# Ighina/MultimodalTopicSegmentation

Hardware: AMD Instinct MI355X
Metric: sentences/sec (fwd+bwd) (higher is better)
Workload: dtype bf16; 1 GPU; BASELINE configs[1]: restricted-window transformer tagger d=1792 heads=8 ff=256 radius=15 layers=1 focal loss, 64 docs x 256 sentences per GPU, fwd+bwd+Adam(eps 1e-7), inputs resident in HBM; global_batch_docs=64, sentences_per_doc=256, parallelism=dp1 (document-sharded, RCCL all-reduce)

## Files before the change

multimodaltopicsegmentation_amd/csrc/gemm.hip:

```cpp
#include <algorithm>
#include <math.h>
#include <stdlib.h>
#include "common.h"

#include "gemm_common.h"


template <int LAYOUT, typename TC, bool GLDS>
__global__ __launch_bounds__(256, 2) void gemm_bf16_kernel(const GemmArgs a) {
  constexpr bool A_KMAJOR = (LAYOUT == MTS_NT || LAYOUT == MTS_NN);
  constexpr bool B_KMAJOR = (LAYOUT == MTS_NT || LAYOUT == MTS_TT);
  extern __shared__ __attribute__((aligned(16))) char smem[];

  const int tid = threadIdx.x;
  const int lane = tid & 63;
  const int wave = tid >> 6;
  const int wm = wave >> 1, wn = wave & 1;
  const int r16 = lane & 15, g = lane >> 4;

  const int ntn = (a.N + BN - 1) / BN;
  const int ntm = (a.M + BM - 1) / BM;
  const int nt = ntn * ntm;
  int bid = xcd_remap(blockIdx.x, nt);
  const int bm0 = (ntm < ntn ? bid % ntm : bid / ntn) * BM;
// ... 485 lines not shown
  if (accumulate) load4<float>(C + (size_t)m * ldc + n, s);
  const size_t plane = (size_t)M * N;
  for (int z = 0; z < splits; ++z) {
    float v[4];
    load4<float>(slab + z * plane + (size_t)m * N + n, v);
#pragma unroll
    for (int i = 0; i < 4; ++i) s[i] += v[i];
  }
  store4<float>(C + (size_t)m * ldc + n, s);
}

__global__ __launch_bounds__(256) void splitk_reduce_t_kernel(const float* __restrict__ slab, int splits, int M, int N, float* __restrict__ Ct,
                                                              int ldc, int accumulate) {
  __shared__ float tile[32][33];
  const int n0 = blockIdx.x * 32, m0 = blockIdx.y * 32;
  const int tx = threadIdx.x & 31, ty = threadIdx.x >> 5;
  const size_t plane = (size_t)M * N;
#pragma unroll
  for (int r = ty; r < 32; r += 8) {
    const int m = m0 + r, n = n0 + tx;
    float s = 0.f;
    if (m < M && n < N) {
      const float* p = slab + (size_t)m * N + n;
      int z = 0;
      for (; z + 7 < splits; z += 8) {
        float v[8];
#pragma unroll
        for (int u = 0; u < 8; ++u) v[u] = p[(size_t)(z + u) * plane];
#pragma unroll
        for (int u = 0; u < 8; ++u) s += v[u];
      }
      for (; z < splits; ++z) s += p[(size_t)z * plane];
    }
    tile[r][tx] = s;
  }
  __syncthreads();
#pragma unroll
  for (int r = ty; r < 32; r += 8) {
    const int n = n0 + r, m = m0 + tx;
    if (n < N && m < M) {
      float* o = Ct + (size_t)n * ldc + m;
      *o = accumulate ? *o + tile[tx][r] : tile[tx][r];
    }
  }
}

template <typename T> __global__ void cast_kernel(const float* __restrict__ src, T* __restrict__ dst, size_t n) {
  size_t i = ((size_t)blockIdx.x * blockDim.x + threadIdx.x) * 4;
  const size_t stride = (size_t)gridDim.x * blockDim.x * 4;
  for (; i + 3 < n; i += stride) {
    float v[4];
    load4<float>(src + i, v);
    store4<T>(dst + i, v);
  }
  if (i < n && i + 3 >= n)
    for (size_t j = i; j < n; ++j) dst[j] = from_f32<T>(src[j]);
}

template <typename T> __global__ void cast_concat_kernel(const float* __restrict__ s1, const float* __restrict__ s2, T* __restrict__ dst,
                                                          size_t rows, int D1, int D2) {
  const int D = D1 + D2, q = D / 4;
  const size_t total = rows * q;
  for (size_t i = (size_t)blockIdx.x * blockDim.x + threadIdx.x; i < total; i += (size_t)gridDim.x * blockDim.x) {
    const size_t r = i / q;
    const int e = (int)(i - r * q) * 4;
    float v[4];
    load4<float>(e < D1 ? s1 + r * D1 + e : s2 + r * D2 + (e - D1), v);
    store4<T>(dst + r * D + e, v);
  }
}

extern "C" int mts_cast_concat(void* stream, int dst_dtype, size_t rows, int D1, int D2, const float* src1, const float* src2, void* dst) {
  MTS_CHECK_ARG(src1 && src2 && dst && D1 > 0 && D2 > 0 && D1 % 4 == 0 && D2 % 4 == 0, "mts_cast_concat: bad arguments (widths must be multiples of 4)");
  if (rows == 0) return MTS_OK;
  const int blocks = (int)std::min<size_t>(4096, (rows * ((D1 + D2) / 4) + 255) / 256);
  if (dst_dtype == MTS_BF16) hipLaunchKernelGGL(cast_concat_kernel<bf16_t>, dim3(blocks), dim3(256), 0, (hipStream_t)stream, src1, src2, (bf16_t*)dst, rows, D1, D2);
  else if (dst_dtype == MTS_F32) hipLaunchKernelGGL(cast_concat_kernel<float>, dim3(blocks), dim3(256), 0, (hipStream_t)stream, src1, src2, (float*)dst, rows, D1, D2);
  else { mts_set_error("mts_cast_concat: bad dtype %d", dst_dtype); return MTS_ERR_INVALID; }
  MTS_LAUNCH_CHECK("mts_cast_concat");
  return MTS_OK;
}

extern "C" size_t mts_colsum_workspace(int N) { return (size_t)COLSUM_RS * (size_t)N * sizeof(float); }

extern "C" int mts_colsum(void* stream, int dtype, int M, int N, const void* X, int ldx, float* out, int accumulate,
                          void* partial) {
  MTS_CHECK_ARG(M > 0 && N > 0 && X && out && partial, "mts_colsum: bad arguments");
  MTS_CHECK_ARG(dtype == MTS_F32 || dtype == MTS_BF16, "mts_colsum: bad dtype %d", dtype);
  MTS_CHECK_ARG(ldx % 4 == 0, "mts_colsum: ldx must be a multiple of 4");
  hipStream_t st = (hipStream_t)stream;
  const int nparts = min(COLSUM_RS, M);
  dim3 grid(ceil_div(N, 64), COLSUM_RS);
  (void)nparts;
  if (dtype == MTS_F32)
    hipLaunchKernelGGL(colsum_partial_kernel<float>, grid, dim3(256), 0, st, (const float*)X, M, N, ldx, (float*)partial);
  else
    hipLaunchKernelGGL(colsum_partial_kernel<bf16_t>, grid, dim3(256), 0, st, (const bf16_t*)X, M, N, ldx, (float*)partial);
  hipLaunchKernelGGL(colsum_final_kernel, dim3(ceil_div(N, 64)), dim3(256), 0, st, (const float*)partial, N, COLSUM_RS, out,
                     accumulate);
  MTS_LAUNCH_CHECK("mts_colsum");
  return MTS_OK;
}

extern "C" int mts_cast(void* stream, int dst_dtype, const float* src, void* dst, size_t n) {
  MTS_CHECK_ARG(src && dst, "mts_cast: null pointer");
  if (n == 0) return MTS_OK;
  hipStream_t st = (hipStream_t)stream;
  const int blocks = (int)std::min<size_t>(2048, (n / 4 + 255) / 256 + 1);
  if (dst_dtype == MTS_BF16)
    hipLaunchKernelGGL(cast_kernel<bf16_t>, dim3(blocks), dim3(256), 0, st, src, (bf16_t*)dst, n);
  else if (dst_dtype == MTS_F32)
    hipLaunchKernelGGL(cast_kernel<float>, dim3(blocks), dim3(256), 0, st, src, (float*)dst, n);
  else {
    mts_set_error("mts_cast: bad dtype %d", dst_dtype);
    return MTS_ERR_INVALID;
  }
  MTS_LAUNCH_CHECK("mts_cast");
  return MTS_OK;
}

int mts_launch_gemm256(const GemmArgs& a, int layout, bool c_is_f32, int splits, hipStream_t st);
int mts_launch_gemm224(const GemmArgs& a, int layout, bool c_is_f32, int splits, hipStream_t st);
bool mts_gemm224t_applies(const GemmArgs& a, int layout, bool c_is_f32, int splits);

static thread_local int g_gemm_glds = -1;
static thread_local int g_tile_mode = -1;
static thread_local int g_force_splits = 0;
static thread_local int g_tile_order = 1;
static thread_local int g_gemm_deep = 1;
static thread_local int g_chain = 0;
static thread_local int g_combine = 0;
#define MTS_GEMM_WS_HEAD 8192
static thread_local int g_last_tile = 0, g_last_splits = 0;

static thread_local void (*g_mid_hook)(void) = nullptr;
extern "C" int mts_gemm_set_mid_hook(void (*fn)(void)) { g_mid_hook = fn; return MTS_OK; }

extern "C" int mts_gemm_last_plan(int* tile, int* splits) {
  if (tile) *tile = g_last_tile;
  if (splits) *splits = g_last_splits;
  return MTS_OK;
}

void mts_band_set_mfma(int on);
void mts_band_set_fused(int on);
void mts_full_set_mfma(int on);
void mts_t5_set_mfma(int on);
static thread_local int g_f32_mfma = 1;
static thread_local int g_big_min_k = 256;
static thread_local int g_gemm_variant = 0;
void mts_lstm_pair_set_spin_limit(int n);
void mts_lstm_pair_set_max_pairs(int n);
void mts_lstm_pair_set_parts(int n);
extern "C" int mts_set_option(const char* key, int value) {
  if (!key) return MTS_ERR_INVALID;
  if (!strcmp(key, "gemm_tile")) { g_tile_mode = value; return MTS_OK; }
  if (!strcmp(key, "gemm_glds")) { g_gemm_glds = value; return MTS_OK; }
  if (!strcmp(key, "gemm_splits")) { g_force_splits = value; return MTS_OK; }
  if (!strcmp(key, "gemm_order")) { g_tile_order = value; return MTS_OK; }
  if (!strcmp(key, "gemm_chain")) { g_chain = value; return MTS_OK; }
  if (!strcmp(key, "gemm_combine")) { g_combine = value; return MTS_OK; }
  if (!strcmp(key, "gemm_deep")) { g_gemm_deep = value; return MTS_OK; }
  if (!strcmp(key, "gemm_variant")) { g_gemm_variant = value; return MTS_OK; }
  if (!strcmp(key, "gemm_big_min_k")) { g_big_min_k = value; return MTS_OK; }
  if (!strcmp(key, "gemm_f32_mfma")) { g_f32_mfma = value; return MTS_OK; }
  if (!strcmp(key, "band_mfma")) { mts_band_set_mfma(value); return MTS_OK; }
  if (!strcmp(key, "band_fused_bwd")) { mts_band_set_fused(value); return MTS_OK; }
  if (!strcmp(key, "full_mfma")) { mts_full_set_mfma(value); return MTS_OK; }
  if (!strcmp(key, "t5_mfma")) { mts_t5_set_mfma(value); return MTS_OK; }
  if (!strcmp(key, "lstm_pair_spin_limit")) { mts_lstm_pair_set_spin_limit(value); return MTS_OK; }
  if (!strcmp(key, "lstm_pair_max_pairs")) { mts_lstm_pair_set_max_pairs(value); return MTS_OK; }
  if (!strcmp(key, "lstm_parts")) { mts_lstm_pair_set_parts(value); return MTS_OK; }
  mts_set_error("mts_set_option: unknown key %s", key);
  return MTS_ERR_INVALID;
}

template <int LAYOUT, typename TC>
static void launch_bf16(const GemmArgs& a, int splits, hipStream_t st) {
  const int nt = ceil_div(a.M, BM) * ceil_div(a.N, BN);
  if (g_gemm_glds < 0) {
    const char* e = getenv("MTS_GEMM_GLDS");
    g_gemm_glds = (e && e[0] == '0') ? 0 : 1;
  }
  const bool glds = g_gemm_glds && (a.K % BK == 0) && (a.ksplit % BK == 0) && a.M >= 8 && a.N >= 8;
  if (glds) {
    GemmArgs b = a;
    const bool deep = g_gemm_deep && (size_t)nt * splits <= 256 && a.ksplit >= 4 * BK;
    b.nbuf = deep ? 4 : 2;
    auto k = gemm_bf16_kernel<LAYOUT, TC, true>;
    if (deep && mts_dyn_lds(k, 8 * TILE_BYTES, "gemm") != MTS_OK) b.nbuf = 2;
    hipLaunchKernelGGL(k, dim3(nt, 1, splits), dim3(256), (b.nbuf == 4 ? 8 : 4) * TILE_BYTES, st, b);
  } else {
    hipLaunchKernelGGL((gemm_bf16_kernel<LAYOUT, TC, false>), dim3(nt, 1, splits), dim3(256), 4 * TILE_BYTES, st, a);
  }
}

static void plan_bf16(int c_dtype, int layout, int M, int N, int K, unsigned epilogue, bool has_workspace, size_t workspace_bytes,
                      int* use256_out, int* splits_out) {
  if (g_tile_mode < 0) {
    const char* e = getenv("MTS_GEMM_TILE");
    g_tile_mode = e ? atoi(e) : 0;
  }
  const int tile_mode = g_tile_mode;
  const unsigned plain = epilogue & ~MTS_EPI_ACCUM;
  const bool can_split = (c_dtype == MTS_F32 && plain == 0 && has_workspace && N % 4 == 0 && K >= 2048);
  const bool can256 = (K % BK == 0) && K >= g_big_min_k && M >= 8 && N >= 8 && tile_mode != 128;
  const double bw = 3500.0;
  double best = 1e30;
  int splits = 1;
  int use256 = 0;
  const bool can224 = can256 && (N % 224 == 0) && tile_mode != 256;
  for (int big = 0; big <= (can256 ? 2 : 0); ++big) {
    if (big == 2 && !can224) continue;
    if (tile_mode == 256 && can256 && big != 1) continue;
    if (tile_mode == 224 && can224 && big != 2) continue;
    const int tile = big ? 256 : 128;
    const double slots = big ? 256.0 : 512.0;
    const double t_k = layout == MTS_TN ? (big == 2 ? (M % 256 == 0 ? 0.0160 : 0.0200) : big == 1 ? 0.0218 : 0.0145)
                                        : (big ? 0.0232 * (big == 2 ? 0.875 : 1.0) : 0.0180);
    const double t_0 = big ? 7.7 : 6.5;
    const int nt = ceil_div(M, tile) * (big == 2 ? N / 224 : ceil_div(N, tile));
    for (int sp = 1; sp <= (can_split ? 32 : 1); ++sp) {
      const int ks = ceil_div(ceil_div(K, sp), BK) * BK;
      if (ceil_div(K, ks) != sp) continue;
      if (sp > 1 && (size_t)sp * M * N * sizeof(float) > workspace_bytes) break;
      if (g_force_splits > 0 && can_split && sp != g_force_splits) continue;
      const double rounds = ceil((double)nt * sp / slots);
      const double cost = rounds * (ks * t_k + t_0) + (sp > 1 ? (2.0 * sp + 1.0) * M * N * 4.0 / 1e6 / bw : 0.0);
      if (cost < best) { best = cost; splits = sp; use256 = big; }
    }
  }
  *use256_out = use256;
  *splits_out = splits;
}

int mts_gemm224_last_kernel();
int mts_launch_gemm224t_pair(const GemmArgs& a, int splits, const void* A2, const void* B2, float* slab2, hipStream_t st);
bool mts_gemm224t_applies(const GemmArgs& a, int layout, bool c_is_f32, int splits);

static int wgrad_pair_splits(int M, int N, int K, size_t workspace_bytes) {
  if (M % 256 || N % 224 || K % 64 || K < 256) return -1;
  static int cus = 0;
  if (!cus) { int dev = 0; hipDeviceProp_t pr; cus = (hipGetDevice(&dev) == hipSuccess && hipGetDeviceProperties(&pr, dev) == hipSuccess) ? pr.multiProcessorCount : 256; }
  const int nt = (M / 256) * (N / 224);
  int sp = std::max(1, std::min(32, cus / (2 * nt)));
  for (; sp >= 1; --sp) {
    const int ks = ceil_div(ceil_div(K, sp), BK) * BK;
    if (ceil_div(K, ks) != sp) continue;
    if (ks >= 128 && K - (sp - 1) * ks >= 128 && (size_t)2 * sp * M * N * sizeof(float) <= workspace_bytes) return sp;
  }
  return -1;
}
extern "C" size_t mts_wgrad_pair_workspace(int M, int N, int K) {
  const int sp = wgrad_pair_splits(M, N, K, (size_t)-1);
  return sp < 1 ? 0 : (size_t)2 * sp * M * N * sizeof(float);
}
extern "C" int mts_wgrad_pair(void* stream, int M, int N, int K, const void* A1, const void* B1, float* C1, int ldc1, const void* A2, const void* B2,
                              float* C2t, int ldc2t, int lda, int ldb, int accumulate, void* workspace, size_t workspace_bytes) {
  MTS_CHECK_ARG(M > 0 && N > 0 && K > 0 && A1 && B1 && C1 && A2 && B2 && C2t && workspace, "mts_wgrad_pair: bad arguments");
  MTS_CHECK_ARG(ldc1 >= N && ldc2t >= M && ldc1 % 4 == 0, "mts_wgrad_pair: bad output strides");
  const int sp = wgrad_pair_splits(M, N, K, workspace_bytes);
  MTS_UNSUPPORTED(sp >= 1, "mts_wgrad_pair: M=%d N=%d K=%d not covered (M %% 256, N %% 224, K %% 64) or workspace too small", M, N, K);
  hipStream_t st = (hipStream_t)stream;
  GemmArgs a;
  memset(&a, 0, sizeof(a));
  a.A = A1; a.B = B1; a.C = C1;
  a.M = M; a.N = N; a.K = K; a.lda = lda; a.ldb = ldb; a.ldc = ldc1;
  a.epi = 0; a.colscale = 1.0f;
  a.ksplit = ceil_div(ceil_div(K, sp), BK) * BK;
  a.order = 1; a.nbuf = 2; a.variant = 0;
  float* const planes = (float*)workspace;
  a.slab = planes;
  float* const planes2 = planes + (size_t)sp * M * N;
  MTS_UNSUPPORTED(mts_gemm224t_applies(a, MTS_TN, true, sp), "mts_wgrad_pair: operands not covered by the four-wave weight-gradient kernel (alignment / strides)");
  const int rc = mts_launch_gemm224t_pair(a, sp, A2, B2, planes2, st);
  MTS_UNSUPPORTED(rc == MTS_OK, "mts_wgrad_pair: launch refused");
  hipLaunchKernelGGL(splitk_reduce_kernel, dim3((unsigned)(((size_t)M * (N / 4) + 255) / 256)), dim3(256), 0, st, (const float*)planes, sp, M, N, C1, ldc1,
                     accumulate ? 1 : 0);
  hipLaunchKernelGGL(splitk_reduce_t_kernel, dim3(ceil_div(N, 32), ceil_div(M, 32)), dim3(256), 0, st, (const float*)planes2, sp, M, N, C2t, ldc2t,
                     accumulate ? 1 : 0);
  MTS_LAUNCH_CHECK("mts_wgrad_pair");
  return MTS_OK;
}

extern "C" int mts_gemm_plan(int a_dtype, int c_dtype, int layout, int M, int N, int K, unsigned epilogue, size_t workspace_bytes,
                             int* tile, int* splits) {
  MTS_CHECK_ARG(M > 0 && N > 0 && K > 0, "mts_gemm_plan: bad shape M=%d N=%d K=%d", M, N, K);
  MTS_CHECK_ARG(layout == MTS_NT || layout == MTS_NN || layout == MTS_TN || layout == MTS_TT, "mts_gemm_plan: bad layout %d", layout);
  MTS_CHECK_ARG(a_dtype == MTS_F32 || a_dtype == MTS_BF16, "mts_gemm_plan: bad a_dtype %d", a_dtype);
  int use256 = 0, sp = 1;
  const size_t ws_planes = workspace_bytes > MTS_GEMM_WS_HEAD ? workspace_bytes - MTS_GEMM_WS_HEAD : 0;
  if (a_dtype == MTS_BF16) plan_bf16(c_dtype, layout, M, N, K, epilogue, ws_planes > 0, ws_planes, &use256, &sp);
  if (tile) *tile = a_dtype == MTS_F32 ? (g_f32_mfma ? 128 : 64) : use256 == 2 ? 224 : use256 == 1 ? 256 : 128;
  if (splits) *splits = sp;
  return MTS_OK;
}

extern "C" int mts_gemm(void* stream, int a_dtype, int c_dtype, int layout, int M, int N, int K, const void* A, int lda,
                        const void* B, int ldb, void* C, int ldc, const float* bias, const void* residual, int ldr,
                        void* aux, int ldaux, unsigned epilogue, float colscale, int ncols_scaled, void* workspace, size_t workspace_bytes) {
  MTS_CHECK_ARG(M > 0 && N > 0 && K > 0, "mts_gemm: bad shape M=%d N=%d K=%d", M, N, K);
  MTS_CHECK_ARG(A && B && C, "mts_gemm: null operand");
  MTS_CHECK_ARG(layout == MTS_NT || layout == MTS_NN || layout == MTS_TN || layout == MTS_TT, "mts_gemm: bad layout %d", layout);
  MTS_CHECK_ARG(a_dtype == MTS_F32 || a_dtype == MTS_BF16, "mts_gemm: bad a_dtype %d", a_dtype);
  MTS_CHECK_ARG(c_dtype == MTS_F32 || c_dtype == a_dtype, "mts_gemm: c_dtype must be f32 or a_dtype");
  MTS_CHECK_ARG(!(epilogue & MTS_EPI_BIAS) || bias, "mts_gemm: MTS_EPI_BIAS without bias");
  MTS_CHECK_ARG(!(epilogue & MTS_EPI_RESIDUAL) || residual, "mts_gemm: MTS_EPI_RESIDUAL without residual");
  MTS_CHECK_ARG(!(epilogue & MTS_EPI_ACCUM) || c_dtype == MTS_F32, "mts_gemm: MTS_EPI_ACCUM needs fp32 C");
// ... 102 lines not shown
```

multimodaltopicsegmentation_amd/csrc/norm.hip:

```cpp
#include <algorithm>
#include <type_traits>
#include "common.h"
#include "loss_elems.h"

#define ROW_WAVES 4
#define BWD_MAX_BLOCKS 512

template <typename T, int NV> struct RowRegs {
  float v[NV][4];
  __device__ __forceinline__ void load(const T* row, int D, int lane) {
#pragma unroll
    for (int i = 0; i < NV; ++i) {
      const int e = 4 * (lane + 64 * i);
      if (e < D) load4<T>(row + e, v[i]);
      else { v[i][0] = v[i][1] = v[i][2] = v[i][3] = 0.f; }
    }
  }
  __device__ __forceinline__ void store(T* row, int D, int lane) const {
#pragma unroll
    for (int i = 0; i < NV; ++i) {
      const int e = 4 * (lane + 64 * i);
      if (e < D) store4<T>(row + e, v[i]);
    }
  }
  __device__ __forceinline__ void zero() {
#pragma unroll
    for (int i = 0; i < NV; ++i) v[i][0] = v[i][1] = v[i][2] = v[i][3] = 0.f;
  }
};

template <int NV> __device__ __forceinline__ void row_stats(const float (&x)[NV][4], int D, int lane, float& mean, float& rstd, float eps) {
  float s = 0.f;
#pragma unroll
  for (int i = 0; i < NV; ++i) s += (x[i][0] + x[i][1]) + (x[i][2] + x[i][3]);
  mean = wave_sum(s) / (float)D;
  float q = 0.f;
#pragma unroll
  for (int i = 0; i < NV; ++i) {
    if (4 * (lane + 64 * i) < D) {
#pragma unroll
      for (int j = 0; j < 4; ++j) { const float d = x[i][j] - mean; q += d * d; }
    }
  }
  rstd = 1.0f / sqrtf(wave_sum(q) / (float)D + eps);
}

template <typename T, int NV, int EMBED, bool FULL = false>
__global__ __launch_bounds__(64 * ROW_WAVES) void ln_fwd_kernel(
    const void* __restrict__ xin, const float* __restrict__ pos, int pos_offset, int L, const float* __restrict__ type0,
    const float* __restrict__ gamma, const float* __restrict__ beta, float eps, int rows, int D,
    T* __restrict__ y, T* __restrict__ pre, float* __restrict__ mean_out, float* __restrict__ rstd_out,
    const float* __restrict__ head_w, const float* __restrict__ head_b, int n_out, float* __restrict__ scores,
    const int32_t* __restrict__ row_src, const float* __restrict__ xin2 = nullptr, int D1 = 0) {
  const int lane = threadIdx.x & 63;
  const int row = blockIdx.x * ROW_WAVES + (threadIdx.x >> 6);
  if (row >= rows) return;
  float gv[NV][4], bv[NV][4];
#pragma unroll
  for (int i = 0; i < NV; ++i) {
    const int e = 4 * (lane + 64 * i);
    if (FULL || e < D) { load4<float>(gamma + e, gv[i]); load4<float>(beta + e, bv[i]); }
  }
  float x[NV][4];
  if constexpr (EMBED) {
    const int src = row_src ? row_src[row] : row;
    const int Dx = xin2 ? D1 : D;
    const float* xr = reinterpret_cast<const float*>(xin) + (size_t)src * Dx;
    const float* xr2 = xin2 ? xin2 + (size_t)src * (D - D1) - D1 : xr;
    const float* pr = pos + (size_t)(pos_offset + src % L) * D;
#pragma unroll
    for (int i = 0; i < NV; ++i) {
      const int e = 4 * (lane + 64 * i);
      if (FULL || e < D) {
        float a[4], b[4], c[4];
        if constexpr (EMBED == 2) load4<bf16_t>(reinterpret_cast<const bf16_t*>(xin) + (size_t)src * D + e, a);
        else load4<float>((e < Dx ? xr : xr2) + e, a);
        load4<float>(pr + e, b); load4<float>(type0 + e, c);
#pragma unroll
        for (int j = 0; j < 4; ++j) x[i][j] = (a[j] + b[j]) + c[j];
        if constexpr (sizeof(T) == 2) {
#pragma unroll
          for (int j = 0; j < 4; ++j) x[i][j] = to_f32(from_f32<T>(x[i][j]));
        }
      } else { x[i][0] = x[i][1] = x[i][2] = x[i][3] = 0.f; }
    }
    if (pre) {
#pragma unroll
      for (int i = 0; i < NV; ++i) { const int e = 4 * (lane + 64 * i); if (FULL || e < D) store4<T>(pre + (size_t)row * D + e, x[i]); }
    }
  } else {
    const T* xr = reinterpret_cast<const T*>(xin) + (size_t)row * D;
#pragma unroll
    for (int i = 0; i < NV; ++i) {
      const int e = 4 * (lane + 64 * i);
      if (FULL || e < D) load4<T>(xr + e, x[i]);
      else { x[i][0] = x[i][1] = x[i][2] = x[i][3] = 0.f; }
    }
  }
  float mean, rstd;
  row_stats<NV>(x, D, lane, mean, rstd, eps);
  float hs[4] = {0.f, 0.f, 0.f, 0.f};
  const float* hwp = head_w ? head_w : gamma;
  const int hw_max = head_w ? n_out - 1 : 0;
#pragma unroll
  for (int i = 0; i < NV; ++i) {
    const int e = 4 * (lane + 64 * i);
    if (FULL || e < D) {
#pragma unroll
      for (int j = 0; j < 4; ++j) x[i][j] = (x[i][j] - mean) * rstd * gv[i][j] + bv[i][j];
      if (head_w) {
#pragma unroll
        for (int c = 0; c < 4; ++c) {
          float w[4];
          load4<float>(hwp + (size_t)min(c, hw_max) * D + e, w);
#pragma unroll
          for (int j = 0; j < 4; ++j) hs[c] += to_f32(from_f32<T>(x[i][j])) * w[j];
        }
      }
    }
  }
  if (y) {
#pragma unroll
    for (int i = 0; i < NV; ++i) {
      const int e = 4 * (lane + 64 * i);
      if (FULL || e < D) store4<T>(y + (size_t)row * D + e, x[i]);
    }
  }
  if (lane == 0 && mean_out) { mean_out[row] = mean; rstd_out[row] = rstd; }
  if (head_w) {
    for (int c = 0; c < n_out; ++c) {
      const float s = wave_sum(hs[c]);
      if (lane == 0) scores[(size_t)row * n_out + c] = s + head_b[c];
    }
  }
}

template <typename T>
__global__ __launch_bounds__(64 * ROW_WAVES) void head_fwd_kernel(const T* __restrict__ x, int ldx, int rows, int D, int n_out,
                                                                const float* __restrict__ w, const float* __restrict__ b,
                                                                float* __restrict__ scores) {
  const int lane = threadIdx.x & 63;
  const int row = blockIdx.x * ROW_WAVES + (threadIdx.x >> 6);
  if (row >= rows) return;
  float hs[4] = {0.f, 0.f, 0.f, 0.f};
  for (int e = 4 * lane; e < D; e += 256) {
    float xv[4];
    load4<T>(x + (size_t)row * ldx + e, xv);
    for (int c = 0; c < n_out; ++c) {
      float wv[4];
      load4<float>(w + (size_t)c * D + e, wv);
#pragma unroll
      for (int j = 0; j < 4; ++j) hs[c] += xv[j] * wv[j];
    }
  }
  for (int c = 0; c < n_out; ++c) {
    const float s = wave_sum(hs[c]);
    if (lane == 0) scores[(size_t)row * n_out + c] = s + b[c];
  }
}

template <typename T>
__global__ __launch_bounds__(256) void head_bwd_data_kernel(const float* __restrict__ ds, const float* __restrict__ w, int rows, int D,
                                                            int n_out, T* __restrict__ dx, int lddx, int accumulate) {
  const size_t idx = (size_t)blockIdx.x * 256 + threadIdx.x;
  const int per_row = D / 4;
  const size_t total = (size_t)rows * per_row;
  if (idx >= total) return;
  const int row = (int)(idx / per_row);
  const int e = 4 * (int)(idx % per_row);
  float o[4] = {0.f, 0.f, 0.f, 0.f};
  if (accumulate) load4<T>(dx + (size_t)row * lddx + e, o);
  for (int c = 0; c < n_out; ++c) {
    const float s = ds[(size_t)row * n_out + c];
    float wv[4];
    load4<float>(w + (size_t)c * D + e, wv);
#pragma unroll
    for (int j = 0; j < 4; ++j) o[j] += s * wv[j];
  }
  store4<T>(dx + (size_t)row * lddx + e, o);
}

struct EmbArgs { int B, L, Bc, nchunks; const int32_t* row0; const int32_t* lengths; float* dpos_part; };

template <typename T, int NV, bool WIDE, bool FULL = false, int NHG = 0, bool EMB = false>
__global__ __launch_bounds__(64 * ROW_WAVES, 2) void ln_bwd_kernel(
    const T* __restrict__ x, const T* __restrict__ dy_, const float* __restrict__ dlogit, const float* __restrict__ head_w, int n_out,
    const float* __restrict__ gamma, const float* __restrict__ mean, const float* __restrict__ rstd, int rows, int D,
    T* __restrict__ dx, float* __restrict__ partial, const EmbArgs ea) {
  static_assert(!(EMB && (WIDE || NHG > 0)), "the embedding form has no head and D <= 2048");
  constexpr bool HG = NHG > 0;
  constexpr int NR = HG ? NHG + 1 : EMB ? 2 : 3;
  constexpr int NS = HG ? NHG + 2 : NR;
  constexpr int NA = HG ? NHG : 2;
  const T* __restrict__ dy = HG ? nullptr : dy_;
  __shared__ float red[ROW_WAVES][NR][64 * 4];
  __shared__ __attribute__((aligned(16))) float gam_s[NV * 256];
  __shared__ __attribute__((aligned(16))) float hw_s[EMB ? 1 : 4][EMB ? 4 : NV * 256];
  __shared__ __attribute__((aligned(16))) float task_s[EMB ? ROW_WAVES : 1][EMB ? NV * 256 : 4];
  const int lane = threadIdx.x & 63;
  const int wave = __builtin_amdgcn_readfirstlane(threadIdx.x >> 6);
  const int col0 = WIDE ? (int)blockIdx.y * (NV * 256) : 0;
  for (int idx = threadIdx.x; idx < NV * 256; idx += 64 * ROW_WAVES) {
    const int e = col0 + idx;
    gam_s[idx] = (e < D) ? gamma[e] : 0.f;
    if constexpr (!EMB) {
      if (head_w)
        for (int c = 0; c < n_out; ++c) hw_s[c][idx] = (e < D) ? head_w[(size_t)c * D + e] : 0.f;
    }
  }
  __syncthreads();
  float acc[NA][NV][4];
  float dxs[NV][4];
  float tsum[HG ? NHG : 1];
#pragma unroll
  for (int i = 0; i < NV; ++i)
#pragma unroll
    for (int j = 0; j < 4; ++j) {
      dxs[i][j] = 0.f;
#pragma unroll
      for (int c = 0; c < NA; ++c) acc[c][i][j] = 0.f;
    }
#pragma unroll
  for (int c = 0; c < (HG ? NHG : 1); ++c) tsum[c] = 0.f;
  if constexpr (EMB) {
#pragma unroll
    for (int i = 0; i < NV; ++i) *reinterpret_cast<float4*>(&task_s[wave][4 * (lane + 64 * i)]) = make_float4(0.f, 0.f, 0.f, 0.f);
  }

  const float invD = 1.0f / (float)D;
  const int stride = gridDim.x * ROW_WAVES;
  Pack<T, 4> px[NV], pd[HG ? 1 : NV];
  float mu_n = 0.f, rs_n = 0.f, dl_n[4] = {0.f, 0.f, 0.f, 0.f};
  const float* dlp = head_w ? dlogit : mean;
  const int dl_mul = head_w ? n_out : 1, dl_max = head_w ? n_out - 1 : 0;
  auto fetch = [&](int r) {
    mu_n = mean[r];
    rs_n = rstd[r];
    if constexpr (!EMB) {
#pragma unroll
      for (int c = 0; c < 4; ++c) dl_n[c] = dlp[(size_t)r * dl_mul + min(c, dl_max)];
    }
#pragma unroll
    for (int i = 0; i < NV; ++i) {
      const int e = col0 + 4 * (lane + 64 * i);
      if (FULL || e < D) {
        px[i].load(x + (size_t)r * D + e);
        if constexpr (!HG) { if (dy) pd[i].load(dy + (size_t)r * D + e); }
      }
    }
  };
  int task = blockIdx.x * ROW_WAVES + wave;
  int ti = 0, tb = 0, tbend = 0;
  const int ntasks = EMB ? ea.L * ea.nchunks : 0;
  auto row_at = [&](int b, int i) { return ea.row0 ? ea.row0[b] + i : b * ea.L + i; };
  auto valid = [&](int b, int i) { return !ea.row0 || i < ea.lengths[b]; };
  auto open_task = [&](int t) {
    ti = t % ea.L;
    tb = (t / ea.L) * ea.Bc;
    tbend = min(ea.B, tb + ea.Bc);
    while (tb < tbend && !valid(tb, ti)) ++tb;
    return tb < tbend;
  };
  auto write_task = [&](int t) {
    float* o = ea.dpos_part + (size_t)t * D;
#pragma unroll
    for (int i = 0; i < NV; ++i) {
      const int e = 4 * (lane + 64 * i);
      float4* slot = reinterpret_cast<float4*>(&task_s[EMB ? wave : 0][EMB ? e : 0]);
      const float4 v = *slot;
      if (FULL || e < D) *reinterpret_cast<float4*>(o + e) = v;
      *slot = make_float4(0.f, 0.f, 0.f, 0.f);
    }
  };
  auto skip_empty_tasks = [&]() {
    if constexpr (EMB) {
      while (task < ntasks && !open_task(task)) task += stride;
    }
  };
  int row;
  if constexpr (EMB) { skip_empty_tasks(); row = task < ntasks ? row_at(tb, ti) : -1; }
  else row = task < rows ? task : -1;
  if (row >= 0) fetch(row);
  while (row >= 0) {
    const float mu = mu_n, rs = rs_n;
    float xh[NV][4], gy[NV][4];
// ... 516 lines not shown
  float dbs[4] = {0.f, 0.f, 0.f, 0.f};
  Pack<T, 4> px[NV];
  float dl_n[4] = {0.f, 0.f, 0.f, 0.f};
  auto fetch = [&](int r) {
#pragma unroll
    for (int c = 0; c < 4; ++c) dl_n[c] = ds[(size_t)r * n_out + min(c, n_out - 1)];
#pragma unroll
    for (int i = 0; i < NV; ++i) {
      const int e = col0 + 4 * (lane + 64 * i);
      if (FULL || e < D) px[i].load(x + (size_t)r * ldx + e);
    }
  };
  const int stride = gridDim.x * ROW_WAVES;
  int row = blockIdx.x * ROW_WAVES + wave;
  if (row < rows) fetch(row);
  for (; row < rows; row += stride) {
    float dl[4], xv[NV][4];
#pragma unroll
    for (int c = 0; c < 4; ++c) dl[c] = (c < n_out) ? dl_n[c] : 0.f;
#pragma unroll
    for (int i = 0; i < NV; ++i) {
      const int e = col0 + 4 * (lane + 64 * i);
#pragma unroll
      for (int j = 0; j < 4; ++j) xv[i][j] = (FULL || e < D) ? px[i].get(j) : 0.f;
    }
    if (row + stride < rows) fetch(row + stride);
#pragma unroll
    for (int c = 0; c < 4; ++c) dbs[c] += dl[c];
#pragma unroll
    for (int i = 0; i < NV; ++i)
#pragma unroll
      for (int c = 0; c < 4; ++c)
#pragma unroll
        for (int j = 0; j < 4; ++j) dw[c][i][j] += dl[c] * xv[i][j];
  }
  float* slab = partial + (size_t)blockIdx.x * 5 * D;
#pragma unroll
  for (int i = 0; i < NV; ++i) {
    __syncthreads();
#pragma unroll
    for (int c = 0; c < 4; ++c)
#pragma unroll
      for (int j = 0; j < 4; ++j) red[wave][c][lane * 4 + j] = dw[c][i][j];
    __syncthreads();
    for (int t = threadIdx.x; t < 4 * 256; t += 64 * ROW_WAVES) {
      const int slot = t / 256, col = t % 256;
      const int e = col0 + 256 * i + col;
      if (e < D) {
        float s = 0.f;
#pragma unroll
        for (int w = 0; w < ROW_WAVES; ++w) s += red[w][slot][col];
        slab[(size_t)slot * D + e] = s;
      }
    }
  }
  __syncthreads();
  if (lane == 0)
    for (int c = 0; c < 4; ++c) red[wave][c][0] = dbs[c];
  __syncthreads();
  if (threadIdx.x < 4) {
    float s = 0.f;
    for (int w = 0; w < ROW_WAVES; ++w) s += red[w][threadIdx.x][0];
    slab[(size_t)4 * D + threadIdx.x] = s;
  }
}

#define SR_COLS 32
struct SlabOuts { float* o[6]; int short_slot, short_len; const float* alt; int alt_slot, alt_nb; };
__global__ __launch_bounds__(256) void slab_reduce_kernel(const float* __restrict__ partial, int nblocks, int nslots, int D, const SlabOuts so) {
  __shared__ float4 red[32][8];
  const int c4 = threadIdx.x & 7, grp = threadIdx.x >> 3;
  const int e = blockIdx.x * SR_COLS + 4 * c4;
  const int slot = blockIdx.y;
  float* o = so.o[slot];
  if (!o) return;
  if (slot == so.alt_slot) { partial = so.alt - (size_t)slot * D; nblocks = so.alt_nb; nslots = 1; }
  const int len = (slot == so.short_slot) ? so.short_len : D;
  float4 s = make_float4(0.f, 0.f, 0.f, 0.f);
  if (e < len) {
    const float* p = partial + (size_t)slot * D + e;
    const size_t bs = (size_t)nslots * D;
    int b = grp;
    for (; b + 32 * 7 < nblocks; b += 32 * 8) {
      float4 v[8];
#pragma unroll
      for (int u = 0; u < 8; ++u) v[u] = *reinterpret_cast<const float4*>(p + (size_t)(b + 32 * u) * bs);
#pragma unroll
      for (int u = 0; u < 8; ++u) { s.x += v[u].x; s.y += v[u].y; s.z += v[u].z; s.w += v[u].w; }
    }
    for (; b < nblocks; b += 32) {
      const float4 v = *reinterpret_cast<const float4*>(p + (size_t)b * bs);
      s.x += v.x; s.y += v.y; s.z += v.z; s.w += v.w;
    }
  }
  red[grp][c4] = s;
  __syncthreads();
  if (grp == 0 && e < len) {
    float4 t = red[0][c4];
#pragma unroll
    for (int gidx = 1; gidx < 32; ++gidx) { const float4 v = red[gidx][c4]; t.x += v.x; t.y += v.y; t.z += v.z; t.w += v.w; }
    if (e + 3 < len) *reinterpret_cast<float4*>(o + e) = t;
    else { const float tv[4] = {t.x, t.y, t.z, t.w}; for (int j = 0; j < 4 && e + j < len; ++j) o[e + j] = tv[j]; }
  }
}

int mts_slab_reduce_rows(hipStream_t st, const float* partial, int nblocks, int D, float* out) {
  SlabOuts so = {{out, nullptr, nullptr, nullptr, nullptr, nullptr}, -1, 0, nullptr, -1, 0};
  hipLaunchKernelGGL(slab_reduce_kernel, dim3(ceil_div(D, SR_COLS), 1), dim3(256), 0, st, partial, nblocks, 1, D, so);
  MTS_LAUNCH_CHECK("slab_reduce");
  return MTS_OK;
}

template <typename T>
__global__ __launch_bounds__(256) void embed_bwd_kernel(const T* __restrict__ dpre, int B, int L, int D, float* __restrict__ dpos, int pos_offset,
                                                        const int32_t* __restrict__ row0, const int32_t* __restrict__ lengths) {
  const size_t idx = (size_t)blockIdx.x * 256 + threadIdx.x;
  const int per_row = D / 4;
  if (idx >= (size_t)L * per_row) return;
  const int i = (int)(idx / per_row), e = 4 * (int)(idx % per_row);
  float s[4] = {0.f, 0.f, 0.f, 0.f};
  int b = 0;
  if (row0) {
    for (; b < B; ++b) {
      if (i < lengths[b]) {
        float v[4];
        load4<T>(dpre + ((size_t)row0[b] + i) * D + e, v);
#pragma unroll
        for (int j = 0; j < 4; ++j) s[j] += v[j];
      }
    }
  }
  for (; b + 7 < B; b += 8) {
    float v[8][4];
#pragma unroll
    for (int u = 0; u < 8; ++u) load4<T>(dpre + ((size_t)(b + u) * L + i) * D + e, v[u]);
#pragma unroll
    for (int u = 0; u < 8; ++u)
#pragma unroll
      for (int j = 0; j < 4; ++j) s[j] += v[u][j];
  }
  for (; b < B; ++b) {
    float v[4];
    load4<T>(dpre + ((size_t)b * L + i) * D + e, v);
#pragma unroll
    for (int j = 0; j < 4; ++j) s[j] += v[j];
  }
  float* o = dpos + (size_t)(pos_offset + i) * D + e;
  float cur[4];
  load4<float>(o, cur);
#pragma unroll
  for (int j = 0; j < 4; ++j) cur[j] += s[j];
  store4<float>(o, cur);
}
static inline int pick_nv(int D) {
  const int need = ceil_div(D, 256);
  if (need <= 1) return 1;
  if (need <= 2) return 2;
  if (need <= 4) return 4;
  if (need == 7) return 7;
  if (need <= 8) return 8;
  if (need <= 16) return 16;
  return 0;
}

template <typename F> static inline void dispatch_nv(int nv, F&& f) {
  switch (nv) {
    case 1: f(std::integral_constant<int, 1>{}); break;
    case 2: f(std::integral_constant<int, 2>{}); break;
    case 4: f(std::integral_constant<int, 4>{}); break;
    case 7: f(std::integral_constant<int, 7>{}); break;
    case 8: f(std::integral_constant<int, 8>{}); break;
    default: f(std::integral_constant<int, 16>{}); break;
  }
}
template <typename F> static inline void dispatch_nv8(int nv, F&& f) {
  switch (nv) {
    case 1: f(std::integral_constant<int, 1>{}); break;
    case 2: f(std::integral_constant<int, 2>{}); break;
    case 4: f(std::integral_constant<int, 4>{}); break;
    case 7: f(std::integral_constant<int, 7>{}); break;
    default: f(std::integral_constant<int, 8>{}); break;
  }
}

template <typename T, int EMBED>
static int ln_fwd_launch(hipStream_t st, const void* x, const float* pos, int pos_offset, int L, const float* type0, const float* gamma,
                         const float* beta, float eps, int rows, int D, void* y, void* pre, float* mean, float* rstd,
                         const float* head_w, const float* head_b, int n_out, float* scores, const int32_t* row_src = nullptr,
                         const float* x2 = nullptr, int D1 = 0) {
  const int nv = pick_nv(D);
  MTS_UNSUPPORTED(nv > 0 && D % 4 == 0, "layernorm: D=%d must be a multiple of 4 and <= 4096", D);
  dim3 grid(ceil_div(rows, ROW_WAVES)), block(64 * ROW_WAVES);
  dispatch_nv(nv, [&](auto nvc) {
    constexpr int NV = decltype(nvc)::value;
    if (D == NV * 256)
      hipLaunchKernelGGL((ln_fwd_kernel<T, NV, EMBED, true>), grid, block, 0, st, x, pos, pos_offset, L, type0, gamma, beta, eps, rows, D, (T*)y,
                         (T*)pre, mean, rstd, head_w, head_b, n_out, scores, row_src, x2, D1);
    else
      hipLaunchKernelGGL((ln_fwd_kernel<T, NV, EMBED>), grid, block, 0, st, x, pos, pos_offset, L, type0, gamma, beta, eps, rows, D, (T*)y,
                         (T*)pre, mean, rstd, head_w, head_b, n_out, scores, row_src, x2, D1);
  });
  MTS_LAUNCH_CHECK("layernorm_fwd");
  return MTS_OK;
}

static int embed_ln_fwd(void* stream, int dtype, int B, int L, int D, const float* x, const float* x2, int D1, const float* pos, int pos_offset,
                        const float* type0, const float* gamma, const float* beta, float eps, void* y, void* pre, float* mean, float* rstd,
                        const int32_t* row_src, int n_rows, const char* who) {
  MTS_CHECK_ARG(B > 0 && L > 0 && D > 0 && x && pos && type0 && gamma && beta && y, "%s: bad arguments", who);
  MTS_CHECK_ARG(!row_src || (n_rows > 0 && n_rows <= B * L), "%s: packed form needs 0 < n_rows <= B*L", who);
  MTS_CHECK_ARG(!x2 || (D1 > 0 && D1 < D && D1 % 4 == 0), "%s: the first part's width must be a multiple of 4 inside (0, D)", who);
  const int rows = row_src ? n_rows : B * L;
  if (dtype == MTS_F32)
    return ln_fwd_launch<float, 1>((hipStream_t)stream, x, pos, pos_offset, L, type0, gamma, beta, eps, rows, D, y, pre, mean, rstd,
                                      nullptr, nullptr, 0, nullptr, row_src, x2, D1);
  if (dtype == MTS_BF16)
    return ln_fwd_launch<bf16_t, 1>((hipStream_t)stream, x, pos, pos_offset, L, type0, gamma, beta, eps, rows, D, y, pre, mean, rstd,
                                       nullptr, nullptr, 0, nullptr, row_src, x2, D1);
  mts_set_error("%s: bad dtype %d", who, dtype);
  return MTS_ERR_INVALID;
}

extern "C" int mts_embed_layernorm_fwd(void* stream, int dtype, int B, int L, int D, const float* x, const float* pos, int pos_offset,
                                       const float* type0, const float* gamma, const float* beta, float eps, void* y, void* pre,
                                       float* mean, float* rstd, const int32_t* row_src, int n_rows) {
  return embed_ln_fwd(stream, dtype, B, L, D, x, nullptr, 0, pos, pos_offset, type0, gamma, beta, eps, y, pre, mean, rstd, row_src, n_rows,
                      "mts_embed_layernorm_fwd");
}

extern "C" int mts_embed_layernorm_fwd_x16(void* stream, int B, int L, int D, const void* x_bf16, const float* pos, int pos_offset, const float* type0,
                                           const float* gamma, const float* beta, float eps, void* y, void* pre, float* mean, float* rstd,
                                           const int32_t* row_src, int n_rows) {
  MTS_CHECK_ARG(B > 0 && L > 0 && D > 0 && x_bf16 && pos && type0 && gamma && beta && y, "mts_embed_layernorm_fwd_x16: bad arguments");
  MTS_CHECK_ARG(!row_src || (n_rows > 0 && n_rows <= B * L), "mts_embed_layernorm_fwd_x16: packed form needs 0 < n_rows <= B*L");
  MTS_CHECK_ARG(((uintptr_t)x_bf16 & 7) == 0, "mts_embed_layernorm_fwd_x16: x must be 8-byte aligned");
  const int rows = row_src ? n_rows : B * L;
  return ln_fwd_launch<bf16_t, 2>((hipStream_t)stream, x_bf16, pos, pos_offset, L, type0, gamma, beta, eps, rows, D, y, pre, mean, rstd, nullptr, nullptr, 0,
                                  nullptr, row_src, nullptr, 0);
}

extern "C" int mts_embed_layernorm_fwd2(void* stream, int dtype, int B, int L, int D1, int D2, const float* x1, const float* x2, const float* pos,
                                        int pos_offset, const float* type0, const float* gamma, const float* beta, float eps, void* y, void* pre,
                                        float* mean, float* rstd, const int32_t* row_src, int n_rows) {
  MTS_CHECK_ARG(x2 && D2 > 0 && D2 % 4 == 0, "mts_embed_layernorm_fwd2: second part missing or its width not a multiple of 4");
  return embed_ln_fwd(stream, dtype, B, L, D1 + D2, x1, x2, D1, pos, pos_offset, type0, gamma, beta, eps, y, pre, mean, rstd, row_src, n_rows,
                      "mts_embed_layernorm_fwd2");
}

extern "C" int mts_layernorm_fwd(void* stream, int dtype, int rows, int D, const void* x, const float* gamma, const float* beta, float eps,
                                 void* y, float* mean, float* rstd, const float* head_w, const float* head_b, int n_out, float* scores) {
  MTS_CHECK_ARG(rows > 0 && D > 0 && x && gamma && beta && (y || (head_w && mean && rstd)), "mts_layernorm_fwd: bad arguments (y may be NULL only with a fused head and saved statistics)");
  MTS_CHECK_ARG(!head_w || (head_b && scores && n_out >= 1 && n_out <= 4), "mts_layernorm_fwd: fused head needs head_b, scores, n_out<=4");
  if (dtype == MTS_F32)
    return ln_fwd_launch<float, 0>((hipStream_t)stream, x, nullptr, 0, 1, nullptr, gamma, beta, eps, rows, D, y, nullptr, mean, rstd,
                                       head_w, head_b, n_out, scores);
  if (dtype == MTS_BF16)
    return ln_fwd_launch<bf16_t, 0>((hipStream_t)stream, x, nullptr, 0, 1, nullptr, gamma, beta, eps, rows, D, y, nullptr, mean, rstd,
                                        head_w, head_b, n_out, scores);
  mts_set_error("mts_layernorm_fwd: bad dtype %d", dtype);
  return MTS_ERR_INVALID;
}

extern "C" size_t mts_layernorm_bwd_workspace(int D) { return (size_t)BWD_MAX_BLOCKS * 6 * (size_t)D * sizeof(float); }

template <typename T>
static int ln_bwd_launch(hipStream_t st, int rows, int D, const void* x, const void* dy, const float* dlogit, const float* head_w, int n_out,
                         const float* gamma, const float* beta, const float* mean, const float* rstd, void* dx, float* dgamma, float* dbeta,
                         float* dxsum, float* dhead_w, float* dhead_b, void* partial) {
  const int nv = pick_nv(D);
  MTS_UNSUPPORTED(nv > 0 && D % 4 == 0, "layernorm_bwd: D=%d must be a multiple of 4 and <= 4096", D);
  const int blocks = std::min(BWD_MAX_BLOCKS, ceil_div(rows, ROW_WAVES));
  const int nhg = dhead_w ? n_out : 0;
  const EmbArgs ea = {0, 0, 0, 0, nullptr, nullptr, nullptr};
  auto go = [&](auto k, dim3 grid) {
    hipLaunchKernelGGL(k, grid, dim3(64 * ROW_WAVES), 0, st, (const T*)x, (const T*)dy, dlogit, head_w, n_out, gamma, mean, rstd, rows, D,
                       (T*)dx, (float*)partial, ea);
  };
  if (nv <= 8) {
    dispatch_nv8(nv, [&](auto nvc) {
      constexpr int NV = decltype(nvc)::value;
      if (D == NV * 256) {
        if (nhg == 1) go(ln_bwd_kernel<T, NV, false, true, 1>, dim3(blocks));
        else if (nhg == 2) go(ln_bwd_kernel<T, NV, false, true, 2>, dim3(blocks));
        else go(ln_bwd_kernel<T, NV, false, true>, dim3(blocks));
      } else {
        if (nhg == 1) go(ln_bwd_kernel<T, NV, false, false, 1>, dim3(blocks));
        else if (nhg == 2) go(ln_bwd_kernel<T, NV, false, false, 2>, dim3(blocks));
        else go(ln_bwd_kernel<T, NV, false>, dim3(blocks));
      }
    });
  } else {
    if (nhg == 1) go(ln_bwd_kernel<T, 8, true, false, 1>, dim3(blocks, ceil_div(D, 2048)));
    else if (nhg == 2) go(ln_bwd_kernel<T, 8, true, false, 2>, dim3(blocks, ceil_div(D, 2048)));
    else go(ln_bwd_kernel<T, 8, true>, dim3(blocks, ceil_div(D, 2048)));
  }
  if (nhg == 1)
    hipLaunchKernelGGL(ln_head_final_kernel<1>, dim3(ceil_div(D, 32)), dim3(256), 0, st, (const float*)partial, blocks, D, head_w, gamma, beta, dgamma,
                       dbeta, dxsum, dhead_w, dhead_b, (const float*)nullptr, (float*)nullptr);
  else if (nhg == 2)
    hipLaunchKernelGGL(ln_head_final_kernel<2>, dim3(ceil_div(D, 32)), dim3(256), 0, st, (const float*)partial, blocks, D, head_w, gamma, beta, dgamma,
                       dbeta, dxsum, dhead_w, dhead_b, (const float*)nullptr, (float*)nullptr);
  else {
    SlabOuts so = {{dgamma, dbeta, dxsum, nullptr, nullptr, nullptr}, -1, 0, nullptr, -1, 0};
    hipLaunchKernelGGL(slab_reduce_kernel, dim3(ceil_div(D, SR_COLS), 3), dim3(256), 0, st, (const float*)partial, blocks, 3, D, so);
  }
  MTS_LAUNCH_CHECK("layernorm_bwd");
  return MTS_OK;
}

extern "C" int mts_layernorm_bwd(void* stream, int dtype, int rows, int D, const void* x, const void* dy, const float* dlogit,
                                 const float* head_w, int n_out, const float* gamma, const float* mean, const float* rstd, void* dx,
                                 float* dgamma, float* dbeta, float* dxsum, void* partial, const float* beta, float* dhead_w, float* dhead_b) {
  MTS_CHECK_ARG(rows > 0 && D > 0 && x && gamma && mean && rstd && dx && partial, "mts_layernorm_bwd: bad arguments");
  MTS_CHECK_ARG(dy || head_w, "mts_layernorm_bwd: needs dy and/or a fused head gradient");
  MTS_CHECK_ARG(!head_w || (dlogit && n_out >= 1 && n_out <= 4), "mts_layernorm_bwd: fused head needs dlogit, n_out<=4");
  MTS_CHECK_ARG(!dhead_w || (head_w && beta && dhead_b && n_out <= 2 && !dy),
                "mts_layernorm_bwd: head parameter gradients need head_w, beta, dhead_b, n_out <= 2 and dy == NULL (the last layer)");
  if (dtype == MTS_F32)
    return ln_bwd_launch<float>((hipStream_t)stream, rows, D, x, dy, dlogit, head_w, n_out, gamma, beta, mean, rstd, dx, dgamma, dbeta, dxsum, dhead_w, dhead_b, partial);
  if (dtype == MTS_BF16)
    return ln_bwd_launch<bf16_t>((hipStream_t)stream, rows, D, x, dy, dlogit, head_w, n_out, gamma, beta, mean, rstd, dx, dgamma, dbeta, dxsum, dhead_w, dhead_b, partial);
  mts_set_error("mts_layernorm_bwd: bad dtype %d", dtype);
  return MTS_ERR_INVALID;
}

extern "C" int mts_layernorm_loss_tail_supported(int dtype, int D, int n_out) {
  return (dtype == MTS_F32 || dtype == MTS_BF16) && (n_out == 1 || n_out == 2) && D % 256 == 0 &&
         (D == 256 || D == 512 || D == 1024 || D == 1792 || D == 2048);
}

template <typename T>
static int ln_tail_launch(hipStream_t st, int rows, int D, const void* x, const float* gamma, const float* beta, float eps, const float* head_w,
                          const float* head_b, int n_out, void* dx, float* dgamma, float* dbeta, float* dxsum, float* dhead_w, float* dhead_b,
                          float* ws, const TailArgs& ta0) {
  const int nv = D / 256;
  const int blocks = std::min(BWD_MAX_BLOCKS, ceil_div(rows, ROW_WAVES));
  TailArgs ta = ta0;
  ta.loss_part = ws + (size_t)BWD_MAX_BLOCKS * 5 * D;
  dispatch_nv8(nv, [&](auto nvc) {
    constexpr int NV = decltype(nvc)::value;
    if (n_out == 1)
      hipLaunchKernelGGL((ln_tail_kernel<T, NV, 1>), dim3(blocks), dim3(64 * ROW_WAVES), 0, st, (const T*)x, gamma, beta, eps, head_w, head_b, rows, D, (T*)dx, ws, ta);
    else
      hipLaunchKernelGGL((ln_tail_kernel<T, NV, 2>), dim3(blocks), dim3(64 * ROW_WAVES), 0, st, (const T*)x, gamma, beta, eps, head_w, head_b, rows, D, (T*)dx, ws, ta);
  });
// ... 205 lines not shown
```

Before: 9.457 million sentences/s.

## Add position-walk embedding layernorm kernel that stages pos/gamma/beta in LDS

Adds a persistent forward kernel for the embedding+layernorm step. Each block handles one sentence position across a chunk of documents, so the position row, gamma, beta and type vectors are loaded once into shared memory and reused. The next row's input is prefetched while the current row is normalised. It is enabled by default when the embedding path has no row_src or head, and it adds LDS use and register pressure for D=1792 (NV=7).

```diff
diff --git a/multimodaltopicsegmentation_amd/csrc/gemm.hip b/multimodaltopicsegmentation_amd/csrc/gemm.hip
--- a/multimodaltopicsegmentation_amd/csrc/gemm.hip
+++ b/multimodaltopicsegmentation_amd/csrc/gemm.hip
@@ -661,8 +661,12 @@
 void mts_lstm_pair_set_spin_limit(int n);
 void mts_lstm_pair_set_max_pairs(int n);
 void mts_lstm_pair_set_parts(int n);
+void mts_norm_set_embed_walk(int on);
+void mts_norm_set_embed_walk_chunk(int n);
 extern "C" int mts_set_option(const char* key, int value) {
   if (!key) return MTS_ERR_INVALID;
+  if (!strcmp(key, "embed_walk")) { mts_norm_set_embed_walk(value); return MTS_OK; }
+  if (!strcmp(key, "embed_walk_chunk")) { mts_norm_set_embed_walk_chunk(value); return MTS_OK; }
   if (!strcmp(key, "gemm_tile")) { g_tile_mode = value; return MTS_OK; }
   if (!strcmp(key, "gemm_glds")) { g_gemm_glds = value; return MTS_OK; }
   if (!strcmp(key, "gemm_splits")) { g_force_splits = value; return MTS_OK; }
diff --git a/multimodaltopicsegmentation_amd/csrc/norm.hip b/multimodaltopicsegmentation_amd/csrc/norm.hip
--- a/multimodaltopicsegmentation_amd/csrc/norm.hip
+++ b/multimodaltopicsegmentation_amd/csrc/norm.hip
@@ -131,6 +131,92 @@
     for (int c = 0; c < n_out; ++c) {
       const float s = wave_sum(hs[c]);
       if (lane == 0) scores[(size_t)row * n_out + c] = s + head_b[c];
+    }
+  }
+}
+
+struct WalkArgs { int B, L, Bc, ntasks; };
+
+template <typename T, int NV, int EMBED, bool FULL = false>
+__global__ __launch_bounds__(64 * ROW_WAVES, FULL ? 4 : 3) void ln_fwd_walk_kernel(
+    const void* __restrict__ xin, const float* __restrict__ pos, int pos_offset, const float* __restrict__ type0,
+    const float* __restrict__ gamma, const float* __restrict__ beta, float eps, int D,
+    T* __restrict__ y, T* __restrict__ pre, float* __restrict__ mean_out, float* __restrict__ rstd_out,
+    const float* __restrict__ xin2, int D1, const WalkArgs wa) {
+  static_assert(EMBED == 1 || EMBED == 2, "the walk is the embedding block's");
+  using XT = std::conditional_t<EMBED == 2, bf16_t, float>;
+  __shared__ __attribute__((aligned(16))) float gam_s[NV * 256];
+  __shared__ __attribute__((aligned(16))) float bet_s[NV * 256];
+  __shared__ __attribute__((aligned(16))) float typ_s[NV * 256];
+  __shared__ __attribute__((aligned(16))) float pos_s[NV * 256];
+  const int lane = threadIdx.x & 63;
+  const int wave = __builtin_amdgcn_readfirstlane(threadIdx.x >> 6);
+  for (int idx = threadIdx.x; idx < NV * 256; idx += 64 * ROW_WAVES) {
+    const bool in = FULL || idx < D;
+    gam_s[idx] = in ? gamma[idx] : 0.f;
+    bet_s[idx] = in ? beta[idx] : 0.f;
+    typ_s[idx] = in ? type0[idx] : 0.f;
+  }
+  const int Dx = xin2 ? D1 : D;
+  Pack<XT, 4> px[NV];
+  auto fetch_x = [&](int src) {
+    const XT* xr = reinterpret_cast<const XT*>(xin) + (size_t)src * Dx;
+    const XT* xr2 = xr;
+    if constexpr (EMBED == 1) { if (xin2) xr2 = xin2 + (size_t)src * (D - D1) - D1; }
+#pragma unroll
+    for (int i = 0; i < NV; ++i) {
+      const int e = 4 * (lane + 64 * i);
+      if (FULL || e < D) px[i].load((e < Dx ? xr : xr2) + e);
+    }
+  };
+  for (int task = blockIdx.x; task < wa.ntasks; task += gridDim.x) {
+    const int ti = task % wa.L, tb0 = (task / wa.L) * wa.Bc, tbend = min(wa.B, tb0 + wa.Bc);
+    int tb = tb0 + wave;
+    if (tb < tbend) fetch_x(tb * wa.L + ti);
+    if (task != (int)blockIdx.x) __syncthreads();
+    const float* pr = pos + (size_t)(pos_offset + ti) * D;
+    for (int idx = threadIdx.x; idx < NV * 256; idx += 64 * ROW_WAVES) pos_s[idx] = (FULL || idx < D) ? pr[idx] : 0.f;
+    __syncthreads();
+    while (tb < tbend) {
+      const int row = tb * wa.L + ti;
+      float x[NV][4];
+#pragma unroll
+      for (int i = 0; i < NV; ++i) {
+        const int e = 4 * (lane + 64 * i);
+        if (FULL || e < D) {
+          const float4 p4v = *reinterpret_cast<const float4*>(pos_s + e), c4v = *reinterpret_cast<const float4*>(typ_s + e);
+          const float b[4] = {p4v.x, p4v.y, p4v.z, p4v.w}, c[4] = {c4v.x, c4v.y, c4v.z, c4v.w};
+#pragma unroll
+          for (int j = 0; j < 4; ++j) x[i][j] = (px[i].get(j) + b[j]) + c[j];
+          if constexpr (sizeof(T) == 2) {
+#pragma unroll
+            for (int j = 0; j < 4; ++j) x[i][j] = to_f32(from_f32<T>(x[i][j]));
+          }
+        } else { x[i][0] = x[i][1] = x[i][2] = x[i][3] = 0.f; }
+        asm volatile("" : "+v"(x[i][0]), "+v"(x[i][1]), "+v"(x[i][2]), "+v"(x[i][3]) :: "memory");
+        __builtin_amdgcn_sched_barrier(0);
+      }
+      tb += ROW_WAVES;
+      if (tb < tbend) fetch_x(tb * wa.L + ti);
+#pragma unroll
+      for (int i = 0; i < NV; ++i) { const int e = 4 * (lane + 64 * i); if (FULL || e < D) store4<T>(pre + (size_t)row * D + e, x[i]); }
+      float mean, rstd;
+      row_stats<NV>(x, D, lane, mean, rstd, eps);
+      asm volatile("" ::: "memory");
+#pragma unroll
+      for (int i = 0; i < NV; ++i) {
+        const int e = 4 * (lane + 64 * i);
+        if (FULL || e < D) {
+          const float4 g4v = *reinterpret_cast<const float4*>(gam_s + e), b4v = *reinterpret_cast<const float4*>(bet_s + e);
+          const float gv[4] = {g4v.x, g4v.y, g4v.z, g4v.w}, bv[4] = {b4v.x, b4v.y, b4v.z, b4v.w};
+#pragma unroll
+          for (int j = 0; j < 4; ++j) x[i][j] = (x[i][j] - mean) * rstd * gv[j] + bv[j];
+          store4<T>(y + (size_t)row * D + e, x[i]);
+        }
+        asm volatile("" ::: "memory");
+        __builtin_amdgcn_sched_barrier(0);
+      }
+      if (lane == 0) { mean_out[row] = mean; rstd_out[row] = rstd; }
     }
   }
 }
@@ -953,6 +1039,12 @@
   for (int j = 0; j < 4; ++j) cur[j] += s[j];
   store4<float>(o, cur);
 }
+static thread_local int g_embed_walk = 1;
+static thread_local int g_embed_walk_chunk = 0;
+void mts_norm_set_embed_walk(int on) { g_embed_walk = on; }
+void mts_norm_set_embed_walk_chunk(int n) { g_embed_walk_chunk = n; }
+#define FWD_WALK_BLOCKS 512
+
 static inline int pick_nv(int D) {
   const int need = ceil_div(D, 256);
   if (need <= 1) return 1;
@@ -992,6 +1084,26 @@
   const int nv = pick_nv(D);
   MTS_UNSUPPORTED(nv > 0 && D % 4 == 0, "layernorm: D=%d must be a multiple of 4 and <= 4096", D);
   dim3 grid(ceil_div(rows, ROW_WAVES)), block(64 * ROW_WAVES);
+  if constexpr (EMBED != 0) {
+    if (g_embed_walk && !row_src && !head_w && nv <= 8 && rows % L == 0 && pre && mean && rstd) {
+      const int B = rows / L;
+      const int C = std::max(1, std::min(ceil_div(B, ROW_WAVES), ceil_div(FWD_WALK_BLOCKS, L)));
+      const int Bc = g_embed_walk_chunk > 0 ? std::min(B, g_embed_walk_chunk) : ceil_div(ceil_div(B, C), ROW_WAVES) * ROW_WAVES;
+      const WalkArgs wa = {B, L, Bc, L * ceil_div(B, Bc)};
+      const dim3 wgrid(std::min(FWD_WALK_BLOCKS, wa.ntasks));
+      dispatch_nv8(nv, [&](auto nvc) {
+        constexpr int NV = decltype(nvc)::value;
+        if (D == NV * 256)
+          hipLaunchKernelGGL((ln_fwd_walk_kernel<T, NV, EMBED, true>), wgrid, block, 0, st, x, pos, pos_offset, type0, gamma, beta, eps, D, (T*)y,
+                             (T*)pre, mean, rstd, x2, D1, wa);
+        else
+          hipLaunchKernelGGL((ln_fwd_walk_kernel<T, NV, EMBED>), wgrid, block, 0, st, x, pos, pos_offset, type0, gamma, beta, eps, D, (T*)y,
+                             (T*)pre, mean, rstd, x2, D1, wa);
+      });
+      MTS_LAUNCH_CHECK("embed_layernorm_fwd");
+      return MTS_OK;
+    }
+  }
   dispatch_nv(nv, [&](auto nvc) {
     constexpr int NV = decltype(nvc)::value;
     if (D == NV * 256)
```

After: 9.518 million sentences/s (median of 6 runs). About the same (+0.6%).
